# wenhe-jia/BM2F

Hardware: AMD Instinct MI355X
Metric: images/sec fwd+bwd, R50 100-query 1024² bs16, at 1/2/4/8 MI355X (higher is better)
Workload: dtype fp16; 1 GPU; config 2: Mask2Former R50 COCO-panoptic, 100 queries, 1024x1024, 16 images/GPU, fwd+bwd+AdamW; pixel decoder + MSDA in fp32 (as the reference forces), backbone/decoder under AMP fp16 with GradScaler; model=maskformer2_R50, global_batch=16, seq_len=21504, queries=100, parallelism=dp1, backbone_layout=channels_last, graph_replay=False

## Files before the change

bm2f_amd/_native.py:

```python
from __future__ import annotations

import contextlib
import ctypes
import os
import threading

import torch

_LIB_PATH = os.path.join(os.path.dirname(os.path.abspath(__file__)), "lib", "libbm2f.so")
_lock = threading.Lock()
_lib = None

ABI_VERSION = 1

_p = ctypes.c_void_p
_i = ctypes.c_int
_f = ctypes.c_float
_l = ctypes.c_int64

_SIGNATURES = {
    "m2f_msda_fwd_f32": [_p, _p, _p, _p, _p, _i, _i, _i, _i, _i, _i, _i, _i, _p, _p, _p],
    "m2f_msda_fwd_f64": [_p, _p, _p, _p, _p, _i, _i, _i, _i, _i, _i, _i, _i, _p, _p, _p],
    "m2f_msda_bwd_f32": [_p, _p, _p, _p, _p, _p, _i, _i, _i, _i, _i, _i, _i, _i, _p, _p, _p, _p, _p],
    "m2f_msda_bwd_f64": [_p, _p, _p, _p, _p, _p, _i, _i, _i, _i, _i, _i, _i, _i, _p, _p, _p, _p, _p],
    "m2f_msda_fused_fwd_f32": [_p, _p, _i, _p, _l, _p, _i, _i, _i, _i, _i, _i, _i, _p, _p],
    "m2f_msda_fused_bwd_workspace": [_p, _i, _i, _i, _i, _i, _i, _p],
    "m2f_msda_fused_bwd_f32": [_p, _p, _i, _p, _l, _p, _p, _i, _i, _i, _i, _i, _i, _i, _p, _p, _p, _l, _p],
    "m2f_msda_fused_fwd_hm_f32": [_p, _p, _i, _p, _l, _p, _i, _i, _i, _i, _i, _i, _i, _p, _p],
    "m2f_msda_fused_bwd_hm_f32": [_p, _p, _i, _p, _l, _p, _p, _i, _i, _i, _i, _i, _i, _i, _p, _p, _p, _l, _p],
    "m2f_attn_mask_bits": [_p, _i, _i, _i, _i, _i, _i, _i, _i, _i, _p, _i, _p],
    "m2f_mask_heads_fwd": [_i, _p, _p, _i, _i, _i, _i, _i, _i, _i, _i, _p, _p, _i, _p],
    "m2f_mask_row_fix": [_p, _i, _i, _i, _p],
    "m2f_mask_heads_bwd_workspace": [_i, _i, _l, _p],
    "m2f_mask_heads_bwd_embed": [_i, _p, _p, _i, _i, _i, _l, _p, _p, _l, _p],
    "m2f_mask_heads_bwd_feats": [_i, _p, _i, _p, _i, _i, _i, _i, _l, _i, _p, _p],
    "m2f_masked_attn_plan": [_i, _i, _i, _i, _p, _p, _p, _p],
    "m2f_masked_attn_fwd": [_i, _p, _p, _p, _p, _i, _i, _i, _i, _i, _i, _i, _i, _f, _p, _p, _p, _l, _p],
    "m2f_masked_attn_bwd": [_i, _p, _p, _p, _p, _p, _p, _p, _i, _i, _i, _i, _i, _i, _i, _i, _f, _p, _p, _p, _p,
                            _l, _p],
    "m2f_gemm_f32_nt": [_p, _l, _p, _l, _p, _i, _p, _l, _p, _l, _i, _i, _i, _p],
    "m2f_gemm_f32_tn_workspace": [_i, _i, _i, _p],
    "m2f_gemm_f32_tn": [_p, _l, _p, _l, _p, _l, _p, _i, _i, _i, _p, _l, _p],
    "m2f_gemm_f32x3_nt_workspace": [_i, _i, _p],
    "m2f_gemm_f32x3_nt": [_p, _l, _p, _l, _i, _p, _i, _p, _l, _p, _l, _i, _i, _i, _p, _l, _p],
    "m2f_gemm_f32x3_nt_add": [_p, _l, _p, _l, _i, _p, _i, _p, _l, _p, _p, _l, _p, _l, _i, _i, _i, _p, _l, _p],
    "m2f_gemm_f32x3_nt_bits": [_p, _l, _p, _l, _i, _p, _i, _p, _p, _l, _p, _l, _i, _i, _i, _p, _l, _p],
    "m2f_gemm_f32x3_nt_rowadd": [_p, _l, _p, _l, _i, _p, _l, _i, _p, _l, _i, _i, _i, _p, _l, _p],
    "m2f_gemm_f32x3_tn_workspace": [_i, _i, _i, _p],
    "m2f_gemm_f32x3_tn": [_p, _l, _p, _l, _p, _l, _p, _i, _i, _i, _p, _l, _p],
    "m2f_conv_f32x3_workspace": [_i, _i, _i, _i, _i, _i, _p],
    "m2f_conv_f32x3": [_p, _p, _p, _p, _i, _i, _i, _i, _i, _i, _i, _p, _l, _p],
    "m2f_conv_f32x3_wgrad": [_p, _p, _p, _p, _i, _i, _i, _i, _i, _i, _p, _l, _p],
    "m2f_conv_x3_io": [_p, _i, _i, _p, _p, _p, _i, _i, _i, _i, _i, _i, _i, _i, _i, _p, _l, _p],
    "m2f_conv_x3_wgrad_io": [_p, _p, _i, _i, _p, _p, _i, _i, _i, _i, _i, _i, _p, _l, _p],
    "m2f_bias_act_nchw": [_p, _p, _p, _l, _i, _l, _i, _i, _p],
    "m2f_relu_bwd_sum": [_p, _i, _p, _p, _l, _i, _p],
    "m2f_upsample2x_add_fwd_f32": [_p, _l, _l, _l, _l, _p, _p, _i, _i, _i, _i, _p],
    "m2f_upsample2x_bwd_f32": [_p, _p, _i, _i, _i, _i, _p],
    "m2f_upsample2x_add_fwd_nhwc_f32": [_p, _l, _p, _p, _i, _i, _i, _i, _p],
    "m2f_upsample2x_bwd_nhwc_f32": [_p, _p, _i, _i, _i, _i, _p],
    "m2f_maxpool3s2_fwd": [_p, _p, _p, _l, _i, _i, _i, _p],
    "m2f_maxpool3s2_bwd": [_p, _p, _p, _l, _i, _i, _i, _p],
    "m2f_maxpool3s2_nhwc": [_i, _p, _p, _p, _i, _i, _i, _i, _i, _p],
    "m2f_stream_copy": [_p, _p, _l, _i, _p],
    "m2f_gather_probe": [_p, _i, _l, _p, _i, _p],
    "m2f_set_option": [ctypes.c_char_p, _l],
    "m2f_get_option": [ctypes.c_char_p, _p],
    "m2f_transpose_f32": [_p, _l, _l, _p, _l, _l, _i, _i, _i, _p],
    "m2f_colsum_workspace": [_l, _i, _p],
    "m2f_colsum": [_i, _p, _l, _i, _p, _l, _p, _p],
    "m2f_sum_to_f32": [_p, _i, _l, _i, _p, _p],
    "m2f_group_norm_workspace": [_i, _i, _i, _l, _p],
    "m2f_group_norm_fwd_f32": [_p, _p, _p, _i, _i, _i, _l, _f, _i, _p, _p, _p, _p, _l, _p],
    "m2f_group_norm_bwd_f32": [_p, _p, _p, _p, _p, _p, _i, _i, _i, _l, _i, _p, _p, _p, _p, _l, _p],
    "m2f_add_layernorm_workspace": [_l, _i, _p],
    "m2f_add_layernorm_fwd_f32": [_p, _p, _p, _p, _l, _i, _f, _p, _p, _p, _p],
    "m2f_add_layernorm_bwd_f32": [_p, _p, _p, _p, _p, _p, _l, _i, _p, _p, _p, _p, _l, _p],
    "m2f_lsap_batched": [_p, _i, _i, _i, _l, _p, _p, _p, _p, _p],
# ... 147 lines not shown
```

bm2f_amd/csrc/gemm_x3.hip:

```cpp
#include "bm2f.h"
#include "common.h"
#include "x3_device.h"

#include <hip/hip_runtime.h>

#include <algorithm>
#include <cstdlib>

namespace {

using namespace m2f_x3;

enum Epi { kNone = 0, kBias = 1, kRelu = 2, kMask = 4, kAdd = 8, kBitsOut = 16, kBitsIn = 32 };

__device__ __forceinline__ unsigned spread4(unsigned byte) {
  unsigned x = byte & 0xffu;
  x = (x | (x << 12)) & 0x000F000Fu;
  x = (x | (x << 6)) & 0x03030303u;
  x = (x | (x << 3)) & 0x11111111u;
  return x;
}


__global__ void __launch_bounds__(256) x3_presplit(const float* __restrict__ B, int64_t ldb, int b_kn, int N, int K,
                                                   int NP, int nchunks, __bf16* __restrict__ Bs) {
  const int64_t t = blockIdx.x * static_cast<int64_t>(blockDim.x) + threadIdx.x;
  if (t >= static_cast<int64_t>(nchunks) * NP) return;
  const int c = static_cast<int>(t / NP), n = static_cast<int>(t - static_cast<int64_t>(c) * NP);
  bf8 pl[3][2];
#pragma unroll
  for (int j = 0; j < 16; ++j) {
    const int k = c * 16 + j;
    float v = 0.f;
    if (n < N && k < K) v = b_kn ? B[static_cast<int64_t>(k) * ldb + n] : B[static_cast<int64_t>(n) * ldb + k];
    __bf16 h, m, l;
    split3(v, h, m, l);
    pl[0][j >> 3][j & 7] = h;
    pl[1][j >> 3][j & 7] = m;
    pl[2][j >> 3][j & 7] = l;
  }
  const int sw = swz(n);
#pragma unroll
  for (int p = 0; p < 3; ++p) {
    bf8* dst = reinterpret_cast<bf8*>(Bs + ((static_cast<int64_t>(c) * 3 + p) * NP + n) * 16);
    dst[sw] = pl[p][0];
    dst[sw ^ 1] = pl[p][1];
  }
}

template <int BN, int NW, int EPI, bool KFULL>
__global__ void __launch_bounds__(64 * NW, 2) x3_nt_kernel(const float* __restrict__ A, int64_t lda,
                                                       const __bf16* __restrict__ Bs, int NP,
                                                       const float* __restrict__ bias,
                                                       const float* __restrict__ mask, int64_t ldm,
                                                       const float* D1, const float* D2, int64_t ldd, int dper,
                                                       uint32_t* bits, float* C, int64_t ldc, int M, int N, int K) {
  constexpr int NT = 64 * NW, BM = 32 * NW, TJ = BN / 32;
  constexpr int PIECES = 3 * BN * 2;
  constexpr int NBL = (PIECES + NT - 1) / NT;
  constexpr int CHUNK = 3 * BN * 16;
  constexpr int EP = 36;
  constexpr int LDS_B = 2 * CHUNK * 2, LDS_E = NW * 32 * EP * 4;
  __shared__ __attribute__((aligned(16))) char smem[LDS_B > LDS_E ? LDS_B : LDS_E];
  __bf16(*sb)[CHUNK] = reinterpret_cast<__bf16(*)[CHUNK]>(smem);

  const int nbn = (N + BN - 1) / BN;
  const int tile = xcd_remap(blockIdx.x, gridDim.x);
  const int bm = tile / nbn, bn = tile % nbn;
  const int m0 = bm * BM, n0 = bn * BN;
  const int tid = threadIdx.x, lane = tid & 63, w = tid >> 6;
  const int li = lane & 31, lh = lane >> 5;
  const int arow = m0 + w * 32 + li;
  const float* ap = A + static_cast<int64_t>(min(arow, M - 1)) * lda + lh * 8;
  const bool arow_ok = arow < M;
  const int nk = (K + kBK - 1) / kBK;

  struct Regs {
    f4 a[2];
    bf8 b[NBL];
  };
  auto gload = [&](Regs& r, int c) {
    const int k = c * kBK + lh * 8;
    const int cc = min(c, nk - 1);
    r.a[0] = *reinterpret_cast<const f4*>(ap + min(k, K - 4) - lh * 8);
    r.a[1] = *reinterpret_cast<const f4*>(ap + min(k + 4, K - 4) - lh * 8);
    const __bf16* bc = Bs + static_cast<int64_t>(cc) * 3 * NP * 16;
#pragma unroll
    for (int u = 0; u < NBL; ++u) {
      const int q = min(tid + u * NT, PIECES - 1);
      const int p = q / (BN * 2), rem = q - p * BN * 2;
      r.b[u] = *reinterpret_cast<const bf8*>(bc + (static_cast<int64_t>(p) * NP + n0) * 16 + rem * 8);
    }
  };
  auto bstore = [&](const Regs& r, int buf) {
#pragma unroll
    for (int u = 0; u < NBL; ++u) {
      const int q = tid + u * NT;
      if (PIECES % NT != 0 && q >= PIECES) continue;
      *reinterpret_cast<bf8*>(&sb[buf][q * 8]) = r.b[u];
    }
  };
  auto asplit = [&](const Regs& r, int c, bf8 (&fa)[3]) {
    const int k = c * kBK + lh * 8;
    float x[8];
#pragma unroll
    for (int e = 0; e < 8; ++e) x[e] = KFULL || k + e < K ? r.a[e >> 2][e & 3] : 0.f;
    split8(x, fa);
  };

  f16v acc[TJ];
#pragma unroll
  for (int j = 0; j < TJ; ++j)
#pragma unroll
    for (int e = 0; e < 16; ++e) acc[j][e] = 0.f;

  const int boff = li * 16 + ((lh ^ swz(li)) * 8);
  auto chunk_mfma = [&](int buf, const bf8 (&fa)[3]) {
    const __bf16* base = &sb[buf][0];
#pragma unroll
    for (int j = 0; j < TJ; ++j) {
      const int off = j * 32 * 16 + boff;
      const bf8 bh = *reinterpret_cast<const bf8*>(base + off);
      const bf8 bmv = *reinterpret_cast<const bf8*>(base + BN * 16 + off);
      const bf8 bl = *reinterpret_cast<const bf8*>(base + 2 * BN * 16 + off);
      f16v x = acc[j];
      x = mfma(fa[2], bh, x);
      x = mfma(fa[1], bmv, x);
      x = mfma(fa[0], bl, x);
      x = mfma(fa[1], bh, x);
      x = mfma(fa[0], bmv, x);
      x = mfma(fa[0], bh, x);
      acc[j] = x;
    }
  };

  Regs r0, r1;
  bf8 fa[3], fb[3];
  gload(r0, 0);
  gload(r1, 1);
// ... 89 lines not shown
          if constexpr ((EPI & kAdd) != 0) {
            x += D1[static_cast<int64_t>(dper ? row % dper : row) * ldd + col + t];
            if (D2) x += D2[static_cast<int64_t>(row) * ldd + col + t];
          }
          C[static_cast<int64_t>(row) * ldc + col + t] = x;
        }
      }
    }
    __builtin_amdgcn_wave_barrier();
    __builtin_amdgcn_fence(__ATOMIC_RELEASE, "wavefront");
    __builtin_amdgcn_fence(__ATOMIC_ACQUIRE, "wavefront");
  }
}

template <int BN, int NW>
int launch_nt(int epi, const float* A, int64_t lda, const __bf16* Bs, int NP, const float* bias, const float* mask,
              int64_t ldm, const float* D1, const float* D2, int64_t ldd, int dper, uint32_t* bits, float* C,
              int64_t ldc, int M, int N, int K, hipStream_t st) {
  constexpr int BM = 32 * NW;
  const int64_t nwg = static_cast<int64_t>((M + BM - 1) / BM) * ((N + BN - 1) / BN);
  if (nwg > 0x7fffffff) return m2f::fail(M2F_EUNSUPPORTED, "m2f_gemm_f32x3_nt: too many tiles");
  const dim3 grid(static_cast<unsigned>(nwg)), block(64 * NW);
  if (!m2f::dispatch_one_of<kNone, kBias, kRelu, kBias | kRelu, kMask, kBias | kMask, kAdd, kBias | kAdd,
                            kRelu | kBitsOut, kBias | kRelu | kBitsOut, kBitsIn, kBias | kBitsIn>(epi, [&](auto e) {
        m2f::dispatch_bool(K % kBK == 0, [&](auto kfull) {
          x3_nt_kernel<BN, NW, e.value, kfull.value><<<grid, block, 0, st>>>(A, lda, Bs, NP, bias, mask, ldm, D1, D2, ldd,
                                                                            dper, bits, C, ldc, M, N, K);
        });
      }))
    return m2f::fail(M2F_EINVAL, "m2f_gemm_f32x3_nt: epilogue %d", epi);
  return m2f::check_launch("m2f_gemm_f32x3_nt");
}

int64_t nt_np(int N) { return (N + 383) / 384 * 384; }

int64_t nt_workspace(int N, int K) {
  const int64_t nchunks = (K + kBK - 1) / kBK;
  return nchunks * 3 * nt_np(N) * 16 * 2;
}

template <int NW, bool MFULL, int CSUM>
__global__ void __launch_bounds__(64 * NW, NW >= 8 ? 1 : 2) x3_tn_kernel(const float* __restrict__ A, int64_t lda,
                                                           const float* __restrict__ B, int64_t ldb, int M, int N1,
                                                           int N2, int rows_per_split, int trans_out,
                                                           float* __restrict__ slab, float* __restrict__ colsum_slab,
                                                           int colsum_b) {
  constexpr int NT = 64 * NW, BN = 256, TJ = BN / 32;
  constexpr int JOBS = BN * 2;
  constexpr int NJ = (JOBS + NT - 1) / NT;
  constexpr int CHUNK = 3 * BN * 16;
  constexpr int EP = 36;
  constexpr int LDS_B = 2 * CHUNK * 2, LDS_E = NW * 32 * EP * 4;
  __shared__ __attribute__((aligned(16))) char smem[LDS_B > LDS_E ? LDS_B : LDS_E];
  __bf16(*sb)[CHUNK] = reinterpret_cast<__bf16(*)[CHUNK]>(smem);

  const int nb1 = (N1 + 32 * NW - 1) / (32 * NW), nb2 = (N2 + BN - 1) / BN;
  const int tiles = nb1 * nb2;
  const int id = xcd_remap(blockIdx.x, gridDim.x);
  const int split = id / tiles, t = id % tiles;
  const int b1 = t / nb2, b2 = t % nb2;
  const int n10 = b1 * 32 * NW, n20 = b2 * BN;
  const int r0 = split * rows_per_split;
  const int r1 = min(M, r0 + rows_per_split);
  const int tid = threadIdx.x, lane = tid & 63, w = tid >> 6;
  const int li = lane & 31, lh = lane >> 5;
  const int acol = min(n10 + w * 32 + li, N1 - 1);
  const float* ap = A + acol;
  const int nk = r1 > r0 ? (r1 - r0 + kBK - 1) / kBK : 0;
  const bool csum_a = CSUM == 1 && b2 == 0;
  const bool csum_b = CSUM == 2 && b1 == 0;

  struct Regs {
    float a[8];
    float b[NJ][8];
  };
  const uint32_t aoff = static_cast<uint32_t>(lh * 8 * lda + acol);
  uint32_t boff8[NJ];
#pragma unroll
  for (int u = 0; u < NJ; ++u) {
    const int job = min(tid + u * NT, JOBS - 1), half = job / BN, col = min(n20 + job % BN, N2 - 1);
// ... 153 lines not shown
      const int job = tid + u * NT;
      if (job < JOBS && job / BN == 1) red[job % BN] = csb[u];
    }
    __syncthreads();
#pragma unroll
    for (int u = 0; u < NJ; ++u) {
      const int job = tid + u * NT, col = n20 + job % BN;
      if (job < JOBS && job / BN == 0 && col < N2)
        colsum_slab[static_cast<int64_t>(split) * N2 + col] = csb[u] + red[job % BN];
    }
  }
}

__global__ void __launch_bounds__(256) x3_slab_reduce(const float* __restrict__ slab, int splits, int64_t n,
                                                      float* __restrict__ out, int64_t ldo, int ncols) {
  const int64_t i = blockIdx.x * static_cast<int64_t>(blockDim.x) + threadIdx.x;
  if (i >= n) return;
  float a0 = 0.f, a1 = 0.f, a2 = 0.f, a3 = 0.f;
  int s = 0;
  for (; s + 3 < splits; s += 4) {
    a0 += slab[(s + 0) * n + i];
    a1 += slab[(s + 1) * n + i];
    a2 += slab[(s + 2) * n + i];
    a3 += slab[(s + 3) * n + i];
  }
  for (; s < splits; ++s) a0 += slab[s * n + i];
  const int64_t r = i / ncols, c = i % ncols;
  out[r * ldo + c] = (a0 + a1) + (a2 + a3);
}

struct TnPlan {
  bool swap;
  int nw;
  int n1, n2;
  int tiles, splits, rows;
};

TnPlan tn_plan(int M, int N1, int N2) {
  TnPlan p;
  p.swap = N2 > N1;
  p.n1 = p.swap ? N2 : N1;
  p.n2 = p.swap ? N1 : N2;
  p.nw = p.n1 % 256 == 0 ? 8 : 4;
  if (const int v = m2f::option(m2f::kOptX3TnNw, 0)) p.nw = v == 3 ? 3 : v == 8 ? 8 : 4;
  p.tiles = ((p.n1 + 32 * p.nw - 1) / (32 * p.nw)) * ((p.n2 + 255) / 256);
  int target = (p.n1 % (32 * p.nw) ? 768 : 512) / (p.nw >= 8 ? 2 : 1);
  target = std::max(1, m2f::option(m2f::kOptX3TnBlocks, target));
  int splits = (target + p.tiles - 1) / p.tiles;
  const int max_splits = (M + 8 * kBK - 1) / (8 * kBK);
  if (splits > max_splits) splits = max_splits;
  p.splits = splits < 1 ? 1 : splits;
  const int r = (M + p.splits - 1) / p.splits;
  p.rows = (r + kBK - 1) / kBK * kBK;
  return p;
}

}

extern "C" int m2f_gemm_f32x3_nt_workspace(int N, int K, int64_t* workspace_bytes) {
  if (N <= 0 || K <= 0) return m2f::fail(M2F_EINVAL, "m2f_gemm_f32x3_nt_workspace: N %d K %d", N, K);
  if (workspace_bytes) *workspace_bytes = nt_workspace(N, K);
  return m2f::ok();
}

namespace {

int nt_impl(const char* fn, const float* A, int64_t lda, const float* B, int64_t ldb, int b_kn, const float* bias,
            int relu, const float* mask, int64_t ldm, const float* D1, const float* D2, int64_t ldd, uint32_t* bits_out,
            const uint32_t* bits_in, int64_t ldbits, float* C, int64_t ldc, int M, int N, int K, void* workspace,
            int64_t workspace_bytes, void* stream, int dper = 0) {
  if (M < 0 || N <= 0 || K <= 0) return m2f::fail(M2F_EINVAL, "%s: M %d N %d K %d", fn, M, N, K);
  if (dper < 0 || (dper && !D1)) return m2f::fail(M2F_EINVAL, "%s: row period %d needs D1", fn, dper);
  if (!A || !B || !C) return m2f::fail(M2F_EINVAL, "%s: null pointer", fn);
  if (K % 4 || lda % 4 || lda < K || ldb < (b_kn ? N : K) || ldc < N || !m2f::aligned(A, 16))
    return m2f::fail(M2F_EINVAL, "%s: K, lda must be multiples of 4 (lda >= K), A 16-byte aligned", fn);
  if (mask && ldm < N) return m2f::fail(M2F_EINVAL, "%s: ldm %lld < N", fn, static_cast<long long>(ldm));
  if (relu && mask) return m2f::fail(M2F_EINVAL, "%s: relu and mask are exclusive", fn);
  if (D2 && !D1) return m2f::fail(M2F_EINVAL, "%s: D2 without D1", fn);
  if (D1 && (relu || mask)) return m2f::fail(M2F_EINVAL, "%s: addends exclude relu and mask", fn);
  if (D1 && (ldd < N || (ldd & 3) || (ldc & 3) || ((N & 3) != 0) || !m2f::aligned(D1, 16) ||
             (D2 && !m2f::aligned(D2, 16)) || !m2f::aligned(C, 16)))
    return m2f::fail(M2F_EINVAL, "%s: addends need ldd >= N, N/ldd/ldc multiples of 4, 16-byte alignment", fn);
  if (bits_out || bits_in) {
    if ((bits_out && bits_in) || (bits_out && !relu) || (bits_in && relu) || mask || D1)
      return m2f::fail(M2F_EINVAL, "%s: bits_out needs relu, bits_in excludes relu; neither with mask or addends", fn);
    if (N % 32 || ldbits < N / 32 || (ldc & 3) || !m2f::aligned(C, 16))
      return m2f::fail(M2F_EINVAL, "%s: mask bits need N %% 32 == 0, ldbits >= N / 32, ldc %% 4 == 0", fn);
  }
  if (!workspace || workspace_bytes < nt_workspace(N, K) || !m2f::aligned(workspace, 16))
    return m2f::fail(M2F_EINVAL, "%s: workspace %lld < %lld (16-byte aligned)", fn,
                     static_cast<long long>(workspace_bytes), static_cast<long long>(nt_workspace(N, K)));
  if (M == 0) return m2f::ok();
  hipStream_t st = static_cast<hipStream_t>(stream);
  const int NP = static_cast<int>(nt_np(N)), nchunks = (K + kBK - 1) / kBK;
  __bf16* Bs = static_cast<__bf16*>(workspace);
  x3_presplit<<<m2f::ceil_div(static_cast<int64_t>(nchunks) * NP, 256), 256, 0, st>>>(B, ldb, b_kn, N, K, NP, nchunks, Bs);
  if (int rc = m2f::check_launch(fn)) return rc;
  const int epi = (bias ? kBias : 0) | (relu ? kRelu : 0) | (mask ? kMask : 0) | (D1 ? kAdd : 0) |
                  (bits_out ? kBitsOut : 0) | (bits_in ? kBitsIn : 0);
  uint32_t* bits = bits_out ? bits_out : const_cast<uint32_t*>(bits_in);
  if (bits) ldm = ldbits;
  int cfg = (N % 128 != 0 && N % 96 == 0) ? 4 : 3;
  cfg = m2f::option(m2f::kOptX3NtCfg, cfg);
  switch (cfg) {
    case 0: return launch_nt<128, 4>(epi, A, lda, Bs, NP, bias, mask, ldm, D1, D2, ldd, dper, bits, C, ldc, M, N, K, st);
    case 1: return launch_nt<96, 4>(epi, A, lda, Bs, NP, bias, mask, ldm, D1, D2, ldd, dper, bits, C, ldc, M, N, K, st);
    case 2: return launch_nt<256, 4>(epi, A, lda, Bs, NP, bias, mask, ldm, D1, D2, ldd, dper, bits, C, ldc, M, N, K, st);
    case 3: return launch_nt<128, 8>(epi, A, lda, Bs, NP, bias, mask, ldm, D1, D2, ldd, dper, bits, C, ldc, M, N, K, st);
    case 4: return launch_nt<96, 8>(epi, A, lda, Bs, NP, bias, mask, ldm, D1, D2, ldd, dper, bits, C, ldc, M, N, K, st);
    default: return m2f::fail(M2F_EINVAL, "%s: config %d", fn, cfg);
  }
}

}

extern "C" int m2f_gemm_f32x3_nt(const float* A, int64_t lda, const float* B, int64_t ldb, int b_kn, const float* bias,
                                 int relu, const float* mask, int64_t ldm, float* C, int64_t ldc, int M, int N, int K,
                                 void* workspace, int64_t workspace_bytes, void* stream) {
  return nt_impl("m2f_gemm_f32x3_nt", A, lda, B, ldb, b_kn, bias, relu, mask, ldm, nullptr, nullptr, 0, nullptr,
                 nullptr, 0, C, ldc, M, N, K, workspace, workspace_bytes, stream);
}

extern "C" int m2f_gemm_f32x3_nt_add(const float* A, int64_t lda, const float* B, int64_t ldb, int b_kn,
                                     const float* bias, int relu, const float* mask, int64_t ldm, const float* D1,
                                     const float* D2, int64_t ldd, float* C, int64_t ldc, int M, int N, int K,
                                     void* workspace, int64_t workspace_bytes, void* stream) {
  return nt_impl("m2f_gemm_f32x3_nt_add", A, lda, B, ldb, b_kn, bias, relu, mask, ldm, D1, D2, ldd, nullptr, nullptr,
                 0, C, ldc, M, N, K, workspace, workspace_bytes, stream);
}

extern "C" int m2f_gemm_f32x3_nt_rowadd(const float* A, int64_t lda, const float* B, int64_t ldb, int b_kn,
                                        const float* R, int64_t ldr, int period, float* C, int64_t ldc, int M, int N,
                                        int K, void* workspace, int64_t workspace_bytes, void* stream) {
  if (!R || period <= 0) return m2f::fail(M2F_EINVAL, "m2f_gemm_f32x3_nt_rowadd: R and a positive period needed");
  return nt_impl("m2f_gemm_f32x3_nt_rowadd", A, lda, B, ldb, b_kn, nullptr, 0, nullptr, 0, R, nullptr, ldr, nullptr,
                 nullptr, 0, C, ldc, M, N, K, workspace, workspace_bytes, stream, period);
}

extern "C" int m2f_gemm_f32x3_nt_bits(const float* A, int64_t lda, const float* B, int64_t ldb, int b_kn,
                                      const float* bias, int relu, uint32_t* bits_out, const uint32_t* bits_in,
                                      int64_t ldbits, float* C, int64_t ldc, int M, int N, int K, void* workspace,
                                      int64_t workspace_bytes, void* stream) {
  if (!bits_out && !bits_in) return m2f::fail(M2F_EINVAL, "m2f_gemm_f32x3_nt_bits: no mask bits");
  return nt_impl("m2f_gemm_f32x3_nt_bits", A, lda, B, ldb, b_kn, bias, relu, nullptr, 0, nullptr, nullptr, 0,
                 bits_out, bits_in, ldbits, C, ldc, M, N, K, workspace, workspace_bytes, stream);
}

extern "C" int m2f_gemm_f32x3_tn_workspace(int M, int N1, int N2, int64_t* workspace_bytes) {
  if (M < 0 || N1 <= 0 || N2 <= 0) return m2f::fail(M2F_EINVAL, "m2f_gemm_f32x3_tn_workspace: bad sizes");
  const TnPlan p = tn_plan(M, N1, N2);
  if (workspace_bytes) *workspace_bytes = static_cast<int64_t>(p.splits) * (static_cast<int64_t>(N1) * N2 + N1) * 4;
  return m2f::ok();
}

extern "C" int m2f_gemm_f32x3_tn(const float* A, int64_t lda, const float* B, int64_t ldb, float* C, int64_t ldc,
                                 float* colsum, int M, int N1, int N2, void* workspace, int64_t workspace_bytes,
                                 void* stream) {
  const char* fn = "m2f_gemm_f32x3_tn";
  if (M < 0 || N1 <= 0 || N2 <= 0) return m2f::fail(M2F_EINVAL, "%s: M %d N1 %d N2 %d", fn, M, N1, N2);
  if ((M > 0 && (!A || !B)) || !C) return m2f::fail(M2F_EINVAL, "%s: null pointer", fn);
  if (lda < N1 || ldb < N2 || ldc < N2) return m2f::fail(M2F_EINVAL, "%s: leading dimensions too small", fn);
  const TnPlan p = tn_plan(M, N1, N2);
  const int64_t need = static_cast<int64_t>(p.splits) * (static_cast<int64_t>(N1) * N2 + N1) * 4;
  if (!workspace || workspace_bytes < need)
    return m2f::fail(M2F_EINVAL, "%s: workspace %lld < %lld", fn, static_cast<long long>(workspace_bytes),
                     static_cast<long long>(need));
  hipStream_t st = static_cast<hipStream_t>(stream);
  float* slab = static_cast<float*>(workspace);
  float* cslab = slab + static_cast<int64_t>(p.splits) * N1 * N2;
  const float* a = p.swap ? B : A;
  const float* b = p.swap ? A : B;
  const int64_t la = p.swap ? ldb : lda, lb = p.swap ? lda : ldb;
  const unsigned grid = static_cast<unsigned>(p.splits * p.tiles);
  if (M > 0) {
    float* cs = colsum ? cslab : nullptr;
    const int csum = colsum ? (p.swap ? 2 : 1) : 0;
    const bool mfull = M % kBK == 0;
    m2f::dispatch_one_of<3, 8, 4>(p.nw == 3 || p.nw == 8 ? p.nw : 4, [&](auto nw) {
      m2f::dispatch_bool(mfull, [&](auto mf) {
        m2f::dispatch_int<0, 2>(csum, [&](auto cs_mode) {
          x3_tn_kernel<nw.value, mf.value, cs_mode.value><<<grid, 64 * nw.value, 0, st>>>(
              a, la, b, lb, M, p.n1, p.n2, p.rows, p.swap ? 1 : 0, slab, cs, p.swap ? 1 : 0);
        });
      });
    });
    if (int rc = m2f::check_launch(fn)) return rc;
  }
  const int64_t n = static_cast<int64_t>(N1) * N2;
  if (M > 0) {
    x3_slab_reduce<<<m2f::ceil_div(n, 256), 256, 0, st>>>(slab, p.splits, n, C, ldc, N2);
    if (int rc = m2f::check_launch(fn)) return rc;
    if (colsum) {
      x3_slab_reduce<<<m2f::ceil_div(N1, 256), 256, 0, st>>>(cslab, p.splits, N1, colsum, N1, N1);
      return m2f::check_launch(fn);
    }
    return m2f::ok();
  }
  if (m2f::zero2d_f32_async(C, ldc, N2, N1, st) != hipSuccess) return m2f::fail(M2F_ELAUNCH, "%s: zero fill", fn);
  if (colsum && m2f::zero_async(colsum, static_cast<size_t>(N1) * 4, st) != hipSuccess)
    return m2f::fail(M2F_ELAUNCH, "%s: memset", fn);
  return m2f::ok();
}
```

bm2f_amd/linear_ops.py:

```python
from __future__ import annotations

import torch
import torch.nn.functional as F
from torch import nn
from torch.autograd import Function

from . import _native


ENGINE = "x3"


def _engine(engine):
    e = engine or ENGINE
    if e not in ("x3", "exact"):
        raise ValueError(f"fp32 GEMM engine {e!r}: expected 'x3' or 'exact'")
    return e


def gemm_nt(a, b, bias=None, relu=False, mask=None, out=None, engine=None, b_kn=False, add=()):
    M, K = a.shape
    N = b.shape[1] if b_kn else b.shape[0]
    if out is None:
        out = torch.empty(M, N, device=a.device, dtype=torch.float32)
    msk = (_native.ptr(mask), mask.stride(0) if mask is not None else 0)
    add = [d for d in add if d is not None]
    if _engine(engine) == "x3":
        ws = _native.workspace("m2f_gemm_f32x3_nt_workspace", N, K, device=a.device, floor=16)
        if add:
            if len(add) > 2 or any(d.shape != (M, N) or d.stride() != add[0].stride() or d.stride(1) != 1
                                   for d in add):
                raise RuntimeError("gemm_nt: addends must be (M, N) row-major tensors with one row stride")
            _native.call("m2f_gemm_f32x3_nt_add", a.data_ptr(), a.stride(0), b.data_ptr(), b.stride(0),
                         1 if b_kn else 0, _native.ptr(bias), 1 if relu else 0, *msk,
                         add[0].data_ptr(), add[1].data_ptr() if len(add) > 1 else None, add[0].stride(0),
                         out.data_ptr(), out.stride(0), M, N, K, ws.data_ptr(), ws.numel(), _native.stream(a))
            return out
        _native.call("m2f_gemm_f32x3_nt", a.data_ptr(), a.stride(0), b.data_ptr(), b.stride(0),
                     1 if b_kn else 0, _native.ptr(bias), 1 if relu else 0, *msk,
                     out.data_ptr(), out.stride(0), M, N, K, ws.data_ptr(), ws.numel(), _native.stream(a))
        return out
    if add:
        raise RuntimeError("gemm_nt: addends need the x3 engine")
    if b_kn:
        b = b.t().contiguous()
    _native.call("m2f_gemm_f32_nt", a.data_ptr(), a.stride(0), b.data_ptr(), b.stride(0), _native.ptr(bias),
                 1 if relu else 0, *msk, out.data_ptr(), out.stride(0), M, N, K, _native.stream(a))
    return out


def gemm_nt_rowadd(a, b, r, period):
    M, K = a.shape
    N = b.shape[0]
    out = torch.empty(M, N, device=a.device, dtype=torch.float32)
    ws = _native.workspace("m2f_gemm_f32x3_nt_workspace", N, K, device=a.device, floor=16)
    _native.call("m2f_gemm_f32x3_nt_rowadd", a.data_ptr(), a.stride(0), b.data_ptr(), b.stride(0), 0,
                 r.data_ptr(), r.stride(0), period, out.data_ptr(), out.stride(0), M, N, K, ws.data_ptr(),
                 ws.numel(), _native.stream(a))
    return out


def gemm_nt_bits(a, b, bias=None, bits_out=None, bits_in=None, b_kn=False):
    M, K = a.shape
    N = b.shape[1] if b_kn else b.shape[0]
    out = torch.empty(M, N, device=a.device, dtype=torch.float32)
    bits = bits_out if bits_out is not None else bits_in
    ws = _native.workspace("m2f_gemm_f32x3_nt_workspace", N, K, device=a.device, floor=16)
    _native.call("m2f_gemm_f32x3_nt_bits", a.data_ptr(), a.stride(0), b.data_ptr(), b.stride(0), 1 if b_kn else 0,
                 _native.ptr(bias), 1 if bits_out is not None else 0, _native.ptr(bits_out), _native.ptr(bits_in),
                 bits.stride(0), out.data_ptr(), out.stride(0), M, N, K, ws.data_ptr(), ws.numel(), _native.stream(a))
    return out


def _relu_bits(x2, w1, b1):
    N = w1.shape[0]
    if ENGINE == "x3" and N % 32 == 0:
        bits = torch.empty(x2.shape[0], N // 32, device=x2.device, dtype=torch.int32)
        return gemm_nt_bits(x2, w1, b1, bits_out=bits), bits
    return gemm_nt(x2, w1, b1, relu=True), None


def _masked_dgrad(g, w2, h, bits):
    if bits is not None:
# ... 144 lines not shown
            p2 = pos.reshape(S, pos.shape[-1])
            if not p2.is_contiguous():
                p2 = p2.contiguous()
            r = gemm_nt(p2, wq, bq)
            proj = gemm_nt_rowadd(s2, wq, r, S)
            ctx.save_for_backward(s2, p2, wv, wq)
        else:
            q2 = (s2.view(src.shape) + pos).view(s2.shape) if pos is not None else s2
            proj = gemm_nt(q2, wq, bq)
            ctx.save_for_backward(s2, q2, wv, wq)
        ctx.in_shape = src.shape
        ctx.has_pos = pos is not None
        ctx.pos_shape = pos.shape if pos is not None else None
        ctx.biases = (bv is not None, bq is not None)
        lead = src.shape[:-1]
        return value.view(*lead, wv.shape[0]), proj.view(*lead, wq.shape[0]), s2.view(src.shape)

    @staticmethod
    def backward(ctx, gvalue, gproj, gpass):
        s2, q2, wv, wq = ctx.saved_tensors
        nig = ctx.needs_input_grad
        gv = _grad_rows(gvalue, torch.empty(s2.shape[0], wv.shape[0], device=s2.device))
        gq = _grad_rows(gproj, torch.empty(s2.shape[0], wq.shape[0], device=s2.device))
        gr = _rows(gpass).contiguous() if gpass is not None else None
        dsrc = dpos = None
        dwq = dbq = None
        if ctx.shared_pos:
            p2 = q2
            N, S = ctx.in_shape[0], ctx.in_shape[1]
            gqs = gq.view(N, S, -1).sum(0)
            if nig[1]:
                dpos = gemm_nt(gqs, wq, b_kn=True).view(ctx.pos_shape)
            if nig[0]:
                t = gemm_nt(gq, wq, b_kn=True, add=(gr,))
                dsrc = gemm_nt(gv, wv, b_kn=True, add=(t,), out=t).view(ctx.in_shape)
            if nig[4] or nig[5]:
                dwq, dbq = gemm_tn(gq, s2, colsum=ctx.biases[1] and nig[5])
                if nig[4]:
                    dwq = dwq + gemm_tn(gqs, p2)[0]
        else:
            if ctx.has_pos and nig[1]:
                dq = gemm_nt(gq, wq, b_kn=True)
                dpos = dq.view(ctx.in_shape)
                if ctx.pos_shape != ctx.in_shape:
                    dpos = dpos.sum(0, keepdim=True)
                if nig[0]:
                    dsrc = gemm_nt(gv, wv, b_kn=True, add=(dq, gr)).view(ctx.in_shape)
            elif nig[0]:
                t = gemm_nt(gq, wq, b_kn=True, add=(gr,))
                dsrc = gemm_nt(gv, wv, b_kn=True, add=(t,), out=t).view(ctx.in_shape)
            if nig[4] or nig[5]:
                dwq, dbq = gemm_tn(gq, q2, colsum=ctx.biases[1] and nig[5])
        dwv, dbv = gemm_tn(gv, s2, colsum=ctx.biases[0] and nig[3]) if (nig[2] or nig[3]) else (None, None)
        return dsrc, dpos, dwv, dbv, dwq, dbq


def residual_fusable(x, *mods) -> bool:
    return ENGINE == "x3" and x.shape[-1] % 4 == 0 and _eligible(x, *mods) and all(
        m.weight.shape[0] % 4 == 0 for m in mods)


def _eligible_wb(x, weight, bias):
    return (x.is_cuda and x.dtype == torch.float32 and x.numel() > 0 and x.shape[-1] % 4 == 0
            and weight.dtype == torch.float32 and weight.dim() == 2 and weight.is_contiguous()
            and weight.shape[0] % 4 == 0 and weight.shape[1] % 4 == 0
            and (bias is None or bias.dtype == torch.float32))


def _eligible(x, *mods):
    return all(_eligible_wb(x, m.weight, m.bias) for m in mods)


def linear(x: torch.Tensor, mod: nn.Linear, relu: bool = False) -> torch.Tensor:
    return linear_wb(x, mod.weight, mod.bias, relu)


def linear_wb(x: torch.Tensor, weight: torch.Tensor, bias, relu: bool = False) -> torch.Tensor:
    if _eligible_wb(x, weight, bias):
        return LinearF32.apply(x, weight, bias, relu)
    y = F.linear(x, weight, bias)
    return F.relu(y) if relu else y


# ... 11 lines not shown
```

include/bm2f.h:

```cpp
#ifndef BM2F_H_
#define BM2F_H_

#include <stdint.h>

#ifdef __cplusplus
extern "C" {
#endif

enum {
  M2F_OK = 0,
  M2F_EINVAL = 1,
  M2F_ELAUNCH = 2,
  M2F_EUNSUPPORTED = 3
};

enum { M2F_F32 = 0, M2F_F16 = 1, M2F_BF16 = 2 };

const char* m2f_last_error(void);
int m2f_abi_version(void);

int m2f_msda_fwd_f32(const float* value, const int64_t* spatial_shapes, const int64_t* level_start_index,
                     const float* sampling_loc, const float* attn_weight,
                     int batch, int spatial_size, int num_heads, int channels,
                     int num_levels, int num_query, int num_point, int im2col_step,
// ... 67 lines not shown
                        int q_row_stride, int kv_row_stride, int mask_words, float scale, void* out,
                        float* lse, void* workspace, int64_t workspace_bytes, void* stream);

int m2f_masked_attn_bwd(int dtype, const void* q, const void* k, const void* v, const uint32_t* bits,
                        const void* out, const void* grad_out, const float* lse, int batch,
                        int num_queries, int num_keys, int num_heads, int head_dim, int q_row_stride,
                        int kv_row_stride, int mask_words, float scale, void* grad_q, void* grad_k,
                        void* grad_v, void* workspace, int64_t workspace_bytes, void* stream);

int m2f_add_layernorm_workspace(int64_t rows, int C, int64_t* workspace_bytes);
int m2f_add_layernorm_fwd_f32(const float* a, const float* b, const float* gamma, const float* beta,
                              int64_t rows, int C, float eps, float* y, float* mean, float* rstd,
                              void* stream);
int m2f_add_layernorm_bwd_f32(const float* grad_y, const float* a, const float* b, const float* gamma,
                              const float* mean, const float* rstd, int64_t rows, int C, float* grad_x,
                              float* grad_gamma, float* grad_beta, void* workspace,
                              int64_t workspace_bytes, void* stream);

int m2f_gemm_f32_nt(const float* A, int64_t lda, const float* B, int64_t ldb, const float* bias, int relu,
                    const float* mask, int64_t ldm, float* C, int64_t ldc, int M, int N, int K, void* stream);
int m2f_gemm_f32_tn_workspace(int M, int N1, int N2, int64_t* workspace_bytes);
int m2f_gemm_f32_tn(const float* A, int64_t lda, const float* B, int64_t ldb, float* C, int64_t ldc,
                    float* colsum, int M, int N1, int N2, void* workspace, int64_t workspace_bytes,
                    void* stream);

int m2f_gemm_f32x3_nt_workspace(int N, int K, int64_t* workspace_bytes);
int m2f_gemm_f32x3_nt(const float* A, int64_t lda, const float* B, int64_t ldb, int b_kn, const float* bias,
                      int relu, const float* mask, int64_t ldm, float* C, int64_t ldc, int M, int N, int K,
                      void* workspace, int64_t workspace_bytes, void* stream);
int m2f_gemm_f32x3_nt_add(const float* A, int64_t lda, const float* B, int64_t ldb, int b_kn, const float* bias,
                          int relu, const float* mask, int64_t ldm, const float* D1, const float* D2, int64_t ldd,
                          float* C, int64_t ldc, int M, int N, int K, void* workspace, int64_t workspace_bytes,
                          void* stream);
int m2f_gemm_f32x3_nt_rowadd(const float* A, int64_t lda, const float* B, int64_t ldb, int b_kn, const float* R,
                             int64_t ldr, int period, float* C, int64_t ldc, int M, int N, int K, void* workspace,
                             int64_t workspace_bytes, void* stream);
int m2f_gemm_f32x3_nt_bits(const float* A, int64_t lda, const float* B, int64_t ldb, int b_kn, const float* bias,
                           int relu, uint32_t* bits_out, const uint32_t* bits_in, int64_t ldbits, float* C,
                           int64_t ldc, int M, int N, int K, void* workspace, int64_t workspace_bytes, void* stream);
int m2f_gemm_f32x3_tn_workspace(int M, int N1, int N2, int64_t* workspace_bytes);
int m2f_gemm_f32x3_tn(const float* A, int64_t lda, const float* B, int64_t ldb, float* C, int64_t ldc,
                      float* colsum, int M, int N1, int N2, void* workspace, int64_t workspace_bytes,
                      void* stream);

int m2f_conv_f32x3_workspace(int N, int Ci, int Co, int H, int W, int ksize, int64_t* workspace_bytes);
int m2f_conv_f32x3(const float* I, const float* W, const float* bias, float* O, int N, int Ci, int Co, int H, int Wd,
                   int ksize, int mode, void* workspace, int64_t workspace_bytes, void* stream);
int m2f_conv_f32x3_wgrad(const float* grad_out, const float* I, float* dW_tck, float* dbias, int N, int Ci, int Co,
                         int H, int Wd, int ksize, void* workspace, int64_t workspace_bytes, void* stream);
int m2f_conv_x3_io(const void* I, int i_dtype, int i_nhwc, const float* W, const float* bias, void* O, int o_dtype,
                   int o_nhwc, int N, int Ci, int Co, int H, int Wd, int ksize, int mode, void* workspace,
                   int64_t workspace_bytes, void* stream);
int m2f_conv_x3_wgrad_io(const float* grad_out, const void* I, int i_dtype, int i_nhwc, float* dW_tck, float* dbias,
                         int N, int Ci, int Co, int H, int Wd, int ksize, void* workspace, int64_t workspace_bytes,
                         void* stream);

int m2f_sum_to_f32(const void* const* srcs, int k, int64_t n, int dtype, float* out, void* stream);

int m2f_bias_act_nchw(void* x, const void* residual, const float* bias, int64_t N, int C, int64_t HW, int dtype,
                      int channels_last, void* stream);

int m2f_relu_bwd_sum(const void* const* grads, int ngrads, const void* y, void* out, int64_t n, int dtype,
                     void* stream);

int m2f_maxpool3s2_fwd(const void* x, void* y, uint8_t* window, int64_t planes, int H, int W, int dtype, void* stream);
int m2f_maxpool3s2_bwd(const void* grad_y, const uint8_t* window, void* grad_x, int64_t planes, int H, int W, int dtype,
// ... 172 lines not shown
```

Measured before the change: 106.4 images/s.

## Fuse two stacked NT GEMMs for source gradient into one dual-K kernel

Adds a dual-operand x3 NT GEMM kernel that runs two products sharing M and N in one K loop (concatenated K from A1/B1 then A2/B2) and adds the residual gradient in the epilogue. The MSDA linear backward now uses it for dsrc instead of two chained GEMMs, which removes one full read and write of the intermediate output and one launch. It also adds an optional BN=288 tile for the TN kernel behind an option value, plus a higher occupancy bound for the dual kernel. The cost is extra per-chunk branching in the load path and a larger presplit workspace.

```diff
diff --git a/bm2f_amd/_native.py b/bm2f_amd/_native.py
--- a/bm2f_amd/_native.py
+++ b/bm2f_amd/_native.py
@@ -44,6 +44,8 @@
     "m2f_gemm_f32x3_nt_workspace": [_i, _i, _p],
     "m2f_gemm_f32x3_nt": [_p, _l, _p, _l, _i, _p, _i, _p, _l, _p, _l, _i, _i, _i, _p, _l, _p],
     "m2f_gemm_f32x3_nt_add": [_p, _l, _p, _l, _i, _p, _i, _p, _l, _p, _p, _l, _p, _l, _i, _i, _i, _p, _l, _p],
+    "m2f_gemm_f32x3_nt2_workspace": [_i, _i, _i, _p],
+    "m2f_gemm_f32x3_nt2": [_p, _l, _p, _l, _i, _i, _p, _l, _p, _l, _i, _i, _p, _p, _l, _p, _l, _i, _i, _p, _l, _p],
     "m2f_gemm_f32x3_nt_bits": [_p, _l, _p, _l, _i, _p, _i, _p, _p, _l, _p, _l, _i, _i, _i, _p, _l, _p],
     "m2f_gemm_f32x3_nt_rowadd": [_p, _l, _p, _l, _i, _p, _l, _i, _p, _l, _i, _i, _i, _p, _l, _p],
     "m2f_gemm_f32x3_tn_workspace": [_i, _i, _i, _p],
diff --git a/bm2f_amd/csrc/gemm_x3.hip b/bm2f_amd/csrc/gemm_x3.hip
--- a/bm2f_amd/csrc/gemm_x3.hip
+++ b/bm2f_amd/csrc/gemm_x3.hip
@@ -6,6 +6,7 @@
 
 #include <algorithm>
 #include <cstdlib>
+#include <type_traits>
 
 namespace {
 
@@ -48,13 +49,15 @@
   }
 }
 
-template <int BN, int NW, int EPI, bool KFULL>
-__global__ void __launch_bounds__(64 * NW, 2) x3_nt_kernel(const float* __restrict__ A, int64_t lda,
+template <int BN, int NW, int EPI, bool KFULL, bool DUAL = false>
+__global__ void __launch_bounds__(64 * NW, DUAL && BN <= 128 ? 4 : 2) x3_nt_kernel(const float* __restrict__ A, int64_t lda,
                                                        const __bf16* __restrict__ Bs, int NP,
                                                        const float* __restrict__ bias,
                                                        const float* __restrict__ mask, int64_t ldm,
                                                        const float* D1, const float* D2, int64_t ldd, int dper,
-                                                       uint32_t* bits, float* C, int64_t ldc, int M, int N, int K) {
+                                                       uint32_t* bits, float* C, int64_t ldc, int M, int N, int K,
+                                                       const float* __restrict__ A2 = nullptr, int64_t lda2 = 0,
+                                                       int K2 = 0) {
   constexpr int NT = 64 * NW, BM = 32 * NW, TJ = BN / 32;
   constexpr int PIECES = 3 * BN * 2;
   constexpr int NBL = (PIECES + NT - 1) / NT;
@@ -72,18 +75,22 @@
   const int li = lane & 31, lh = lane >> 5;
   const int arow = m0 + w * 32 + li;
   const float* ap = A + static_cast<int64_t>(min(arow, M - 1)) * lda + lh * 8;
-  const bool arow_ok = arow < M;
-  const int nk = (K + kBK - 1) / kBK;
+  const float* ap2 = DUAL ? A2 + static_cast<int64_t>(min(arow, M - 1)) * lda2 + lh * 8 : nullptr;
+  const int nk1 = (K + kBK - 1) / kBK;
+  const int nk = nk1 + (DUAL ? (K2 + kBK - 1) / kBK : 0);
 
   struct Regs {
     f4 a[2];
     bf8 b[NBL];
   };
   auto gload = [&](Regs& r, int c) {
-    const int k = c * kBK + lh * 8;
+    const bool second = DUAL && c >= nk1;
+    const float* apc = second ? ap2 : ap;
+    const int Kc = second ? K2 : K;
+    const int k = (second ? c - nk1 : c) * kBK + lh * 8;
     const int cc = min(c, nk - 1);
-    r.a[0] = *reinterpret_cast<const f4*>(ap + min(k, K - 4) - lh * 8);
-    r.a[1] = *reinterpret_cast<const f4*>(ap + min(k + 4, K - 4) - lh * 8);
+    r.a[0] = *reinterpret_cast<const f4*>(apc + min(k, Kc - 4) - lh * 8);
+    r.a[1] = *reinterpret_cast<const f4*>(apc + min(k + 4, Kc - 4) - lh * 8);
     const __bf16* bc = Bs + static_cast<int64_t>(cc) * 3 * NP * 16;
 #pragma unroll
     for (int u = 0; u < NBL; ++u) {
@@ -101,10 +108,12 @@
     }
   };
   auto asplit = [&](const Regs& r, int c, bf8 (&fa)[3]) {
-    const int k = c * kBK + lh * 8;
+    const bool second = DUAL && c >= nk1;
+    const int Kc = second ? K2 : K;
+    const int k = (second ? c - nk1 : c) * kBK + lh * 8;
     float x[8];
 #pragma unroll
-    for (int e = 0; e < 8; ++e) x[e] = KFULL || k + e < K ? r.a[e >> 2][e & 3] : 0.f;
+    for (int e = 0; e < 8; ++e) x[e] = KFULL || k + e < Kc ? r.a[e >> 2][e & 3] : 0.f;
     split8(x, fa);
   };
 
@@ -260,6 +269,22 @@
   return m2f::check_launch("m2f_gemm_f32x3_nt");
 }
 
+template <int BN, int NW>
+int launch_nt2(const float* A1, int64_t lda1, int K1, const float* A2, int64_t lda2, int K2, const __bf16* Bs, int NP,
+               const float* D1, const float* D2, int64_t ldd, float* C, int64_t ldc, int M, int N, hipStream_t st) {
+  constexpr int BM = 32 * NW;
+  const int64_t nwg = static_cast<int64_t>((M + BM - 1) / BM) * ((N + BN - 1) / BN);
+  if (nwg > 0x7fffffff) return m2f::fail(M2F_EUNSUPPORTED, "m2f_gemm_f32x3_nt2: too many tiles");
+  const dim3 grid(static_cast<unsigned>(nwg)), block(64 * NW);
+  m2f::dispatch_bool(D1 != nullptr, [&](auto add) {
+    m2f::dispatch_bool(K1 % kBK == 0 && K2 % kBK == 0, [&](auto kfull) {
+      x3_nt_kernel<BN, NW, add.value ? kAdd : kNone, kfull.value, true><<<grid, block, 0, st>>>(
+          A1, lda1, Bs, NP, nullptr, nullptr, 0, D1, D2, ldd, 0, nullptr, C, ldc, M, N, K1, A2, lda2, K2);
+    });
+  });
+  return m2f::check_launch("m2f_gemm_f32x3_nt2");
+}
+
 int64_t nt_np(int N) { return (N + 383) / 384 * 384; }
 
 int64_t nt_workspace(int N, int K) {
@@ -267,13 +292,15 @@
   return nchunks * 3 * nt_np(N) * 16 * 2;
 }
 
-template <int NW, bool MFULL, int CSUM>
+int nt_cfg(int N) { return m2f::option(m2f::kOptX3NtCfg, (N % 128 != 0 && N % 96 == 0) ? 4 : 3); }
+
+template <int NW, bool MFULL, int CSUM, int BN = 256>
 __global__ void __launch_bounds__(64 * NW, NW >= 8 ? 1 : 2) x3_tn_kernel(const float* __restrict__ A, int64_t lda,
                                                            const float* __restrict__ B, int64_t ldb, int M, int N1,
                                                            int N2, int rows_per_split, int trans_out,
                                                            float* __restrict__ slab, float* __restrict__ colsum_slab,
                                                            int colsum_b) {
-  constexpr int NT = 64 * NW, BN = 256, TJ = BN / 32;
+  constexpr int NT = 64 * NW, TJ = BN / 32;
   constexpr int JOBS = BN * 2;
   constexpr int NJ = (JOBS + NT - 1) / NT;
   constexpr int CHUNK = 3 * BN * 16;
@@ -493,18 +520,22 @@
 struct TnPlan {
   bool swap;
   int nw;
+  int bn;
   int n1, n2;
   int tiles, splits, rows;
 };
 
 TnPlan tn_plan(int M, int N1, int N2) {
   TnPlan p;
-  p.swap = N2 > N1;
+  const int v = m2f::option(m2f::kOptX3TnNw, 0);
+  const bool fits288 = (N1 == 288 && N2 % 256 == 0) || (N2 == 288 && N1 % 256 == 0);
+  p.bn = fits288 && v == 98 ? 288 : 256;
+  p.swap = p.bn == 288 ? N1 == 288 : N2 > N1;
   p.n1 = p.swap ? N2 : N1;
   p.n2 = p.swap ? N1 : N2;
   p.nw = p.n1 % 256 == 0 ? 8 : 4;
-  if (const int v = m2f::option(m2f::kOptX3TnNw, 0)) p.nw = v == 3 ? 3 : v == 8 ? 8 : 4;
-  p.tiles = ((p.n1 + 32 * p.nw - 1) / (32 * p.nw)) * ((p.n2 + 255) / 256);
+  if (v) p.nw = v == 3 ? 3 : v == 8 || p.bn == 288 ? 8 : 4;
+  p.tiles = ((p.n1 + 32 * p.nw - 1) / (32 * p.nw)) * ((p.n2 + p.bn - 1) / p.bn);
   int target = (p.n1 % (32 * p.nw) ? 768 : 512) / (p.nw >= 8 ? 2 : 1);
   target = std::max(1, m2f::option(m2f::kOptX3TnBlocks, target));
   int splits = (target + p.tiles - 1) / p.tiles;
@@ -561,18 +592,60 @@
                   (bits_out ? kBitsOut : 0) | (bits_in ? kBitsIn : 0);
   uint32_t* bits = bits_out ? bits_out : const_cast<uint32_t*>(bits_in);
   if (bits) ldm = ldbits;
-  int cfg = (N % 128 != 0 && N % 96 == 0) ? 4 : 3;
-  cfg = m2f::option(m2f::kOptX3NtCfg, cfg);
-  switch (cfg) {
+  switch (nt_cfg(N)) {
     case 0: return launch_nt<128, 4>(epi, A, lda, Bs, NP, bias, mask, ldm, D1, D2, ldd, dper, bits, C, ldc, M, N, K, st);
     case 1: return launch_nt<96, 4>(epi, A, lda, Bs, NP, bias, mask, ldm, D1, D2, ldd, dper, bits, C, ldc, M, N, K, st);
     case 2: return launch_nt<256, 4>(epi, A, lda, Bs, NP, bias, mask, ldm, D1, D2, ldd, dper, bits, C, ldc, M, N, K, st);
     case 3: return launch_nt<128, 8>(epi, A, lda, Bs, NP, bias, mask, ldm, D1, D2, ldd, dper, bits, C, ldc, M, N, K, st);
     case 4: return launch_nt<96, 8>(epi, A, lda, Bs, NP, bias, mask, ldm, D1, D2, ldd, dper, bits, C, ldc, M, N, K, st);
-    default: return m2f::fail(M2F_EINVAL, "%s: config %d", fn, cfg);
-  }
-}
-
+    default: return m2f::fail(M2F_EINVAL, "%s: config %d", fn, nt_cfg(N));
+  }
+}
+
+}
+
+extern "C" int m2f_gemm_f32x3_nt2_workspace(int N, int K1, int K2, int64_t* workspace_bytes) {
+  if (N <= 0 || K1 <= 0 || K2 <= 0)
+    return m2f::fail(M2F_EINVAL, "m2f_gemm_f32x3_nt2_workspace: N %d K1 %d K2 %d", N, K1, K2);
+  if (workspace_bytes) *workspace_bytes = nt_workspace(N, K1) + nt_workspace(N, K2);
+  return m2f::ok();
+}
+
+extern "C" int m2f_gemm_f32x3_nt2(const float* A1, int64_t lda1, const float* B1, int64_t ldb1, int b1_kn, int K1,
+                                  const float* A2, int64_t lda2, const float* B2, int64_t ldb2, int b2_kn, int K2,
+                                  const float* D1, const float* D2, int64_t ldd, float* C, int64_t ldc, int M, int N,
+                                  void* workspace, int64_t workspace_bytes, void* stream) {
+  const char* fn = "m2f_gemm_f32x3_nt2";
+  if (M < 0 || N <= 0 || K1 <= 0 || K2 <= 0) return m2f::fail(M2F_EINVAL, "%s: M %d N %d K1 %d K2 %d", fn, M, N, K1, K2);
+  if (!A1 || !B1 || !A2 || !B2 || !C) return m2f::fail(M2F_EINVAL, "%s: null pointer", fn);
+  if (K1 % 4 || K2 % 4 || lda1 % 4 || lda2 % 4 || lda1 < K1 || lda2 < K2 || ldb1 < (b1_kn ? N : K1) ||
+      ldb2 < (b2_kn ? N : K2) || ldc < N || !m2f::aligned(A1, 16) || !m2f::aligned(A2, 16))
+    return m2f::fail(M2F_EINVAL, "%s: K1, K2, lda1, lda2 must be multiples of 4 (lda >= K), A1, A2 16-byte aligned", fn);
+  if (D2 && !D1) return m2f::fail(M2F_EINVAL, "%s: D2 without D1", fn);
+  if (D1 && (ldd < N || (ldd & 3) || (ldc & 3) || ((N & 3) != 0) || !m2f::aligned(D1, 16) ||
+             (D2 && !m2f::aligned(D2, 16)) || !m2f::aligned(C, 16)))
+    return m2f::fail(M2F_EINVAL, "%s: addends need ldd >= N, N/ldd/ldc multiples of 4, 16-byte alignment", fn);
+  const int64_t need = nt_workspace(N, K1) + nt_workspace(N, K2);
+  if (!workspace || workspace_bytes < need || !m2f::aligned(workspace, 16))
+    return m2f::fail(M2F_EINVAL, "%s: workspace %lld < %lld (16-byte aligned)", fn,
+                     static_cast<long long>(workspace_bytes), static_cast<long long>(need));
+  if (M == 0) return m2f::ok();
+  hipStream_t st = static_cast<hipStream_t>(stream);
+  const int NP = static_cast<int>(nt_np(N)), nk1 = (K1 + kBK - 1) / kBK, nk2 = (K2 + kBK - 1) / kBK;
+  __bf16* Bs = static_cast<__bf16*>(workspace);
+  x3_presplit<<<m2f::ceil_div(static_cast<int64_t>(nk1) * NP, 256), 256, 0, st>>>(B1, ldb1, b1_kn, N, K1, NP, nk1, Bs);
+  if (int rc = m2f::check_launch(fn)) return rc;
+  x3_presplit<<<m2f::ceil_div(static_cast<int64_t>(nk2) * NP, 256), 256, 0, st>>>(
+      B2, ldb2, b2_kn, N, K2, NP, nk2, Bs + static_cast<int64_t>(nk1) * 3 * NP * 16);
+  if (int rc = m2f::check_launch(fn)) return rc;
+  switch (nt_cfg(N)) {
+    case 0: return launch_nt2<128, 4>(A1, lda1, K1, A2, lda2, K2, Bs, NP, D1, D2, ldd, C, ldc, M, N, st);
+    case 1: return launch_nt2<96, 4>(A1, lda1, K1, A2, lda2, K2, Bs, NP, D1, D2, ldd, C, ldc, M, N, st);
+    case 2: return launch_nt2<256, 4>(A1, lda1, K1, A2, lda2, K2, Bs, NP, D1, D2, ldd, C, ldc, M, N, st);
+    case 3: return launch_nt2<128, 8>(A1, lda1, K1, A2, lda2, K2, Bs, NP, D1, D2, ldd, C, ldc, M, N, st);
+    case 4: return launch_nt2<96, 8>(A1, lda1, K1, A2, lda2, K2, Bs, NP, D1, D2, ldd, C, ldc, M, N, st);
+    default: return m2f::fail(M2F_EINVAL, "%s: config %d", fn, nt_cfg(N));
+  }
 }
 
 extern "C" int m2f_gemm_f32x3_nt(const float* A, int64_t lda, const float* B, int64_t ldb, int b_kn, const float* bias,
@@ -637,14 +710,19 @@
     float* cs = colsum ? cslab : nullptr;
     const int csum = colsum ? (p.swap ? 2 : 1) : 0;
     const bool mfull = M % kBK == 0;
-    m2f::dispatch_one_of<3, 8, 4>(p.nw == 3 || p.nw == 8 ? p.nw : 4, [&](auto nw) {
+    auto launch = [&](auto nw, auto bn) {
       m2f::dispatch_bool(mfull, [&](auto mf) {
         m2f::dispatch_int<0, 2>(csum, [&](auto cs_mode) {
-          x3_tn_kernel<nw.value, mf.value, cs_mode.value><<<grid, 64 * nw.value, 0, st>>>(
+          x3_tn_kernel<nw.value, mf.value, cs_mode.value, bn.value><<<grid, 64 * nw.value, 0, st>>>(
               a, la, b, lb, M, p.n1, p.n2, p.rows, p.swap ? 1 : 0, slab, cs, p.swap ? 1 : 0);
         });
       });
-    });
+    };
+    if (p.bn == 288)
+      launch(std::integral_constant<int, 8>{}, std::integral_constant<int, 288>{});
+    else
+      m2f::dispatch_one_of<3, 8, 4>(p.nw == 3 || p.nw == 8 ? p.nw : 4,
+                                    [&](auto nw) { launch(nw, std::integral_constant<int, 256>{}); });
     if (int rc = m2f::check_launch(fn)) return rc;
   }
   const int64_t n = static_cast<int64_t>(N1) * N2;
diff --git a/bm2f_amd/linear_ops.py b/bm2f_amd/linear_ops.py
--- a/bm2f_amd/linear_ops.py
+++ b/bm2f_amd/linear_ops.py
@@ -49,6 +49,36 @@
     return out
 
 
+def gemm_nt2(a1, b1, a2, b2, b1_kn=False, b2_kn=False, add=(), out=None):
+    M, K1 = a1.shape
+    K2 = a2.shape[1]
+    N = b1.shape[1] if b1_kn else b1.shape[0]
+    if a2.shape[0] != M or (b2.shape[1] if b2_kn else b2.shape[0]) != N:
+        raise RuntimeError("gemm_nt2: the two products must share M and N")
+    add = [d for d in add if d is not None]
+    if len(add) > 2 or any(d.shape != (M, N) or d.stride() != add[0].stride() or d.stride(1) != 1 for d in add):
+        raise RuntimeError("gemm_nt2: addends must be (M, N) row-major tensors with one row stride")
+    if out is None:
+        out = torch.empty(M, N, device=a1.device, dtype=torch.float32)
+    ws = _native.workspace("m2f_gemm_f32x3_nt2_workspace", N, K1, K2, device=a1.device, floor=16)
+    _native.call("m2f_gemm_f32x3_nt2", a1.data_ptr(), a1.stride(0), b1.data_ptr(), b1.stride(0), 1 if b1_kn else 0, K1,
+                 a2.data_ptr(), a2.stride(0), b2.data_ptr(), b2.stride(0), 1 if b2_kn else 0, K2,
+                 add[0].data_ptr() if add else None, add[1].data_ptr() if len(add) > 1 else None,
+                 add[0].stride(0) if add else 0, out.data_ptr(), out.stride(0), M, N, ws.data_ptr(), ws.numel(),
+                 _native.stream(a1))
+    return out
+
+
+GRAD_SRC_STACKED = True
+
+
+def _grad_src(gq, wq, gv, wv, gr):
+    if GRAD_SRC_STACKED:
+        return gemm_nt2(gq, wq, gv, wv, b1_kn=True, b2_kn=True, add=(gr,))
+    t = gemm_nt(gq, wq, b_kn=True, add=(gr,))
+    return gemm_nt(gv, wv, b_kn=True, add=(t,), out=t)
+
+
 def gemm_nt_rowadd(a, b, r, period):
     M, K = a.shape
     N = b.shape[0]
@@ -259,8 +289,7 @@
             if nig[1]:
                 dpos = gemm_nt(gqs, wq, b_kn=True).view(ctx.pos_shape)
             if nig[0]:
-                t = gemm_nt(gq, wq, b_kn=True, add=(gr,))
-                dsrc = gemm_nt(gv, wv, b_kn=True, add=(t,), out=t).view(ctx.in_shape)
+                dsrc = _grad_src(gq, wq, gv, wv, gr).view(ctx.in_shape)
             if nig[4] or nig[5]:
                 dwq, dbq = gemm_tn(gq, s2, colsum=ctx.biases[1] and nig[5])
                 if nig[4]:
@@ -274,8 +303,7 @@
                 if nig[0]:
                     dsrc = gemm_nt(gv, wv, b_kn=True, add=(dq, gr)).view(ctx.in_shape)
             elif nig[0]:
-                t = gemm_nt(gq, wq, b_kn=True, add=(gr,))
-                dsrc = gemm_nt(gv, wv, b_kn=True, add=(t,), out=t).view(ctx.in_shape)
+                dsrc = _grad_src(gq, wq, gv, wv, gr).view(ctx.in_shape)
             if nig[4] or nig[5]:
                 dwq, dbq = gemm_tn(gq, q2, colsum=ctx.biases[1] and nig[5])
         dwv, dbv = gemm_tn(gv, s2, colsum=ctx.biases[0] and nig[3]) if (nig[2] or nig[3]) else (None, None)
diff --git a/include/bm2f.h b/include/bm2f.h
--- a/include/bm2f.h
+++ b/include/bm2f.h
@@ -123,6 +123,11 @@
                           int relu, const float* mask, int64_t ldm, const float* D1, const float* D2, int64_t ldd,
                           float* C, int64_t ldc, int M, int N, int K, void* workspace, int64_t workspace_bytes,
                           void* stream);
+int m2f_gemm_f32x3_nt2_workspace(int N, int K1, int K2, int64_t* workspace_bytes);
+int m2f_gemm_f32x3_nt2(const float* A1, int64_t lda1, const float* B1, int64_t ldb1, int b1_kn, int K1,
+                       const float* A2, int64_t lda2, const float* B2, int64_t ldb2, int b2_kn, int K2,
+                       const float* D1, const float* D2, int64_t ldd, float* C, int64_t ldc, int M, int N,
+                       void* workspace, int64_t workspace_bytes, void* stream);
 int m2f_gemm_f32x3_nt_rowadd(const float* A, int64_t lda, const float* B, int64_t ldb, int b_kn, const float* R,
                              int64_t ldr, int period, float* C, int64_t ldc, int M, int N, int K, void* workspace,
                              int64_t workspace_bytes, void* stream);
```

Result: no change. 106.8 images/s, median of 6 (+0.4%).
